# francescofrontera/flink-jpmml

Measured on AMD Instinct MI355X. Metric: records/sec (whole node) on 1k-tree GBDT PMML at 1/2/4/8 MI355X; p50 latency, higher is better.
Workload: dtype fp32

## Files before the change

### flink_jpmml_amd/config.py

```python

from __future__ import annotations

import dataclasses
import os
from dataclasses import dataclass, field
from typing import Any, Dict, Optional, Sequence

PRECISIONS = ("fp32", "bf16", "fp8")
FALLBACKS = ("host", "warn", "error")


@dataclass
class ScoringConfig:
    batch_size: Optional[int] = None
    """Flush a per-record micro-batch once it holds this many records (``None`` = score each record
    as it arrives, exactly the reference's call pattern)."""
    udf_mode: str = "deferred"
    """How a micro-batched per-record UDF is run: ``deferred`` — exactly once per event, its
    ``predict`` calls resolved when the batch is scored; ``replay`` — capture, batch score, replay
    (the UDF runs twice: pure UDFs that read the score inside ``f`` batch fully)."""
    max_batch_latency_ms: Optional[float] = None
    """Flush a non-empty micro-batch once its oldest record has waited this long (size-or-time
    trigger). ``None`` = size, control message, checkpoint barrier or end of input only."""

# ... 11 lines not shown
    """What happens when a model cannot be lowered to the device: ``host`` — score on the host
    oracle (batched, vectorised) and count ``scoring.host_fallback``; ``warn`` — the same plus one
    WARNING per model; ``error`` — fail the model load (strict production setting)."""

    reason_codes: bool = False
    """Rank a Scorecard's ``reasonCode`` Output fields (rank 1 … 8) on the device when a batch is
    scored with ``outputs=True`` (``FJA_REASON_CODES=1``). Off: such a field does not lower, and the
    Output fields of that model follow ``fallback``. Other models ignore it."""

    entity_ranks: bool = False
    """Rank the entity Output fields of a clustering or k-NN model on the device when a batch is
    scored with ``outputs=True`` (``FJA_ENTITY_RANKS=1``): ``entityId`` / ``clusterId`` / affinity of
    rank 1 … 32, the affinity of a named cluster, the neighbours' ids and distances. Off: such a field
    does not lower, and the Output fields of that model follow ``fallback``. Other models ignore it."""

    knn_classes: bool = False
    """Score the class Output fields of a k-NN classifier on the device when a batch is scored with
    ``outputs=True`` (``FJA_KNN_CLASSES=1``): the predicted label, the vote shares as ``probability``
    and ``top_k``. Off: such a field does not lower, and the Output fields of that model follow
    ``fallback``. Other models ignore it."""

    svm_classes: bool = False
    """Score the class Output fields of an SVM classifier on the device when a batch is scored with
    ``outputs=True`` (``FJA_SVM_CLASSES=1``): the predicted label, the machines' vote shares as
    ``probability`` and ``top_k``. Off: such a field does not lower, and the Output fields of that
    model follow ``fallback``. Other models ignore it."""

    association_rules: bool = False
    """Rank the ``ruleValue`` / ``entityId`` Output fields of an AssociationModel (rank 1 … 8) on the
    device when a batch is scored with ``outputs=True`` (``FJA_ASSOCIATION_RULES=1``). Off: the
    Output fields of such a model are computed on the host, row by row. A document the rule kernel
    cannot take follows ``fallback``. Other models ignore it."""

    host_threads: int = 0
    """Worker threads of the native host tree walk (``fallback="host"`` models, CPU-only ranks,
    direct CPU ``predict_batch``); 0 = ``FJA_HOST_THREADS`` or 1. Results do not depend on it."""

    micro_batch: int = 1 << 19
    """Rows per device kernel launch when a RecordBatch is split (H2D / kernel overlap)."""
    pipeline_depth: int = 3
    """Device input slots of the H2D → kernel ring (copy of batch i+1 overlaps kernel i)."""
    h2d_streams: int = 0
    """Copy streams each micro-batch's host→device transfer is split over (concurrent copy
    engines); 0 = calibrate 1 vs 2 on the first copy and keep the faster (boxes differ)."""
    max_inflight: int = 4
    """Scored batches an operator keeps in flight before it waits for the oldest (backpressure)."""
    metrics_port: int = 0
    """> 0: every rank serves its metrics in the Prometheus text format on ``GET /metrics`` at
    ``metrics_port + rank`` (127.0.0.1) while a job runs (``utils/metrics.py``)."""
    graph_max_rows: int = 16384
    """Micro-batches of at most this many rows run multi-kernel plans (wide NeuralNetworks,
    segmented ensembles, derive pass + model) as one HIP-graph replay per row bucket
    (:mod:`flink_jpmml_amd.runtime.graphs`); 0 = always launch kernel by kernel."""
    device_mirror: bool = False
    """Keep ``[rows]`` device copies of every columnar result (``PredictionBatch.device_out``) next
    to the pinned host scores, so a :class:`~flink_jpmml_amd.parallel.sinks.GatherSink` all-gathers
    them over RCCL without a host round trip (SURVEY §2.6 F5)."""

    cache_capacity: int = 64
    """Exact-key LRU capacity of loaded models per operator instance."""
    async_load: bool = True
    """Parse + lower an added model on a background loader thread (the event path only waits if an
    event needs the model before the load finished)."""

    checkpoint_dir: Optional[str] = None
    watchdog_s: Optional[float] = None
    """Arm a progress watchdog in the distributed loop: abort the rank when no element was processed
    for this long (a peer stuck in a collective cannot be interrupted from Python)."""

    plan_opts: Dict[str, Any] = field(default_factory=dict)
    """Extra lowering options forwarded to :func:`flink_jpmml_amd.runtime.plans.compile_plan`."""

    def __post_init__(self) -> None:
        if self.precision not in PRECISIONS:
            raise ValueError(f"precision must be one of {PRECISIONS}, got {self.precision!r}")
        if self.udf_mode not in ("deferred", "replay"):
            raise ValueError(f"udf_mode must be 'deferred' or 'replay', got {self.udf_mode!r}")
        if self.fallback not in FALLBACKS:
            raise ValueError(f"fallback must be one of {FALLBACKS}, got {self.fallback!r}")
        if self.batch_size is not None and int(self.batch_size) < 1:
            raise ValueError("batch_size must be >= 1")
        if self.max_batch_latency_ms is not None and float(self.max_batch_latency_ms) < 0:
            raise ValueError("max_batch_latency_ms must be >= 0")
        if self.micro_batch < 1 or self.pipeline_depth < 1 or self.max_inflight < 1:
            raise ValueError("micro_batch, pipeline_depth and max_inflight must be >= 1")

    def replace(self, **kw) -> "ScoringConfig":
        return dataclasses.replace(self, **{k: v for k, v in kw.items() if v is not None})

    def lowering_opts(self) -> Dict[str, Any]:
        opts = dict(self.plan_opts)
        if self.precision != "fp32":
            opts.setdefault("precision", self.precision)
        return opts

    def resolve_device(self, local_rank: int = 0):
        if self.device is None:
            return None
        import torch

        if isinstance(self.device, str) and self.device == "auto":
            if not torch.cuda.is_available():
                return None
            dev = torch.device("cuda")
        else:
            dev = torch.device(self.device) if not isinstance(self.device, torch.device) else self.device
        if dev.type != "cuda":
            return None if dev.type == "cpu" else dev
        if self.device_ids is not None:
            return torch.device("cuda", int(self.device_ids[local_rank % len(self.device_ids)]))
        if dev.index is None:
            n = max(1, torch.cuda.device_count())
            return torch.device("cuda", local_rank % n)
        return dev

    @staticmethod
    def from_env(prefix: str = "FJA_", **overrides) -> "ScoringConfig":
        def get(name, conv):
            v = os.environ.get(prefix + name)
            return conv(v) if v not in (None, "") else None

        kw = dict(batch_size=get("BATCH_SIZE", int), max_batch_latency_ms=get("MAX_BATCH_LATENCY_MS", float),
                  device=get("DEVICE", str), precision=get("PRECISION", str), fallback=get("FALLBACK", str),
                  micro_batch=get("MICRO_BATCH", int), cache_capacity=get("CACHE_CAPACITY", int),
                  checkpoint_dir=get("CHECKPOINT_DIR", str), watchdog_s=get("WATCHDOG_S", float),
                  graph_max_rows=get("GRAPH_MAX_ROWS", int), metrics_port=get("METRICS_PORT", int),
                  host_threads=get("HOST_THREADS", int),
                  reason_codes=get("REASON_CODES", lambda v: v.strip().lower() in ("1", "true", "yes", "on")),
                  entity_ranks=get("ENTITY_RANKS", lambda v: v.strip().lower() in ("1", "true", "yes", "on")),
                  knn_classes=get("KNN_CLASSES", lambda v: v.strip().lower() in ("1", "true", "yes", "on")),
                  svm_classes=get("SVM_CLASSES", lambda v: v.strip().lower() in ("1", "true", "yes", "on")),
                  association_rules=get("ASSOCIATION_RULES",
                                        lambda v: v.strip().lower() in ("1", "true", "yes", "on")))
        kw = {k: v for k, v in kw.items() if v is not None}
        kw.update({k: v for k, v in overrides.items() if v is not None})
        return ScoringConfig(**kw)


def merge_config(config: Optional[ScoringConfig], **legacy) -> ScoringConfig:
    base = config if config is not None else ScoringConfig()
    kw = {k: v for k, v in legacy.items() if v is not None}
    if "plan_opts" in kw:
        kw["plan_opts"] = {**base.plan_opts, **kw["plan_opts"]}
    return dataclasses.replace(base, **kw) if kw else base


__all__ = ["FALLBACKS", "PRECISIONS", "ScoringConfig", "merge_config"]
```

### flink_jpmml_amd/ops/_lib.py

```python

from __future__ import annotations

import ctypes
import glob
import logging
import os
import shutil
import subprocess
import threading
import time
from typing import List, Optional

logger = logging.getLogger(__name__)

HERE = os.path.dirname(os.path.abspath(__file__))
CSRC = os.path.join(HERE, "csrc")
LIB_PATH = os.path.join(HERE, "_pmml_kernels.so")
ARCH = os.environ.get("PYTORCH_ROCM_ARCH", "gfx950").split(";")[0] or "gfx950"


class KernelLibraryError(RuntimeError):
    pass


# ... 342 lines not shown
        lib.pmml_gemm_fused_head_launch.restype = ctypes.c_int
        lib.pmml_gemm_fused_head_launch.argtypes = [c_void_p, ctypes.POINTER(GemmArgs), ctypes.POINTER(GemmArgs),
                                                    c_void_p, c_void_p]
        lib.pmml_nn_prep_launch.restype = ctypes.c_int
        lib.pmml_nn_prep_launch.argtypes = [c_void_p, ctypes.POINTER(NnPrepArgs)]
        lib.pmml_knn_launch.restype = ctypes.c_int
        lib.pmml_knn_launch.argtypes = [c_void_p, ctypes.POINTER(KnnArgs), c_void_p, c_void_p, ctypes.c_int,
                                        ctypes.c_int]
        lib.pmml_linear_launch.argtypes = [c_void_p, ctypes.POINTER(LinearArgs)]
        if hasattr(lib, "pmml_mlp_launch"):
            lib.pmml_mlp_launch.argtypes = [c_void_p, ctypes.POINTER(MlpArgs), c_int]
        if hasattr(lib, "pmml_svm_launch"):
            lib.pmml_svm_launch.argtypes = [c_void_p, ctypes.POINTER(SvmArgs), c_int, c_int]
        if hasattr(lib, "pmml_svm_wide_launch"):
            lib.pmml_svm_wide_launch.restype = c_int
            lib.pmml_svm_wide_launch.argtypes = [c_void_p, ctypes.POINTER(SvmWideArgs), c_int, c_int]
        lib.pmml_tree_general_launch.argtypes = [c_void_p, ctypes.POINTER(GenTreeArgs)]
        lib.pmml_tree_general_launch.restype = c_int
        lib.pmml_tree_hybrid_launch.argtypes = [c_void_p, ctypes.POINTER(HybridArgs), c_int, c_int]
        lib.pmml_tree_hybrid_launch.restype = c_int
        lib.pmml_derive_launch.argtypes = [c_void_p, ctypes.POINTER(DeriveArgs)]
        lib.pmml_derive_launch.restype = c_int
        lib.pmml_mask_invalid.argtypes = [c_void_p, c_void_p, c_void_p, c_void_p, c_void_p, c_void_p, c_int]
        lib.pmml_mask_invalid.restype = c_int
        lib.pmml_host_register.argtypes = [c_void_p, ctypes.c_size_t, ctypes.c_uint]
        lib.pmml_host_register.restype = c_int
        lib.pmml_host_unregister.argtypes = [c_void_p]
        lib.pmml_host_unregister.restype = c_int
        lib.pmml_segment_reduce.argtypes = [c_void_p, ctypes.POINTER(SegArgs)]
        lib.pmml_tree_pointer_multi.argtypes = [c_void_p, ctypes.POINTER(MultiTreeArgs), c_int, c_int]
        lib.pmml_tree_pointer_multi.restype = c_int
        lib.pmml_segment_reduce.restype = c_int
        lib.pmml_tree_launch_many.argtypes = [c_void_p, c_void_p, c_void_p, c_int]
        lib.pmml_tree_launch_many.restype = c_int
        lib.pmml_text_rows_count.argtypes = [c_void_p, c_void_p, ctypes.c_longlong, c_void_p]
        lib.pmml_text_rows_count.restype = c_int
        lib.pmml_text_rows_write.argtypes = [c_void_p, c_void_p, ctypes.c_longlong, c_void_p, c_void_p]
        lib.pmml_text_rows_write.restype = c_int
        lib.pmml_text_parse.argtypes = [c_void_p, ctypes.POINTER(TextParseArgs)]
        lib.pmml_text_parse.restype = c_int
        lib.pmml_group_rows.argtypes = [c_void_p, c_void_p, c_int, c_int, c_int, c_void_p, c_int, c_int, c_void_p,
                                        c_void_p, c_void_p]
        lib.pmml_group_rows.restype = c_int
        lib.pmml_ungroup.argtypes = [c_void_p, c_void_p, c_void_p, c_void_p, c_int, c_void_p, c_void_p, c_void_p,
                                     c_void_p]
        lib.pmml_ungroup.restype = c_int
        lib.pmml_group_slice.argtypes = [c_void_p, c_void_p, c_int, c_int, c_int, c_void_p, c_int, c_int, c_void_p,
                                         c_void_p, c_int, c_void_p, c_void_p, c_void_p, c_void_p, c_void_p,
                                         c_void_p, c_void_p, c_void_p, c_void_p]
        lib.pmml_group_slice.restype = c_int
        lib.pmml_tree_launch_grouped.argtypes = [c_void_p, c_void_p, c_int, ctypes.POINTER(GroupedTreeArgs), c_int,
                                                 c_int]
        lib.pmml_tree_launch_grouped.restype = c_int
        lib.pmml_tree_lds_launch.argtypes = [c_void_p, ctypes.POINTER(LdsTreeArgs)]
        lib.pmml_tree_lds_launch.restype = c_int
        lib.pmml_tree_lds_bytes.argtypes = [c_int, c_int, c_int, c_int, c_int]
        lib.pmml_tree_lds_bytes.restype = ctypes.c_longlong
        lib.pmml_csr_expand.argtypes = [c_void_p, ctypes.POINTER(CsrExpandArgs)]
        lib.pmml_csr_expand.restype = c_int
        lib.pmml_csr_expand_rows.argtypes = [c_int]
        lib.pmml_csr_expand_rows.restype = c_int
        lib.pmml_outputs_launch.argtypes = [c_void_p, ctypes.POINTER(OutputArgs)]
        lib.pmml_outputs_launch.restype = c_int
        lib.pmml_outputs_rows.argtypes = [c_int, c_int]
        lib.pmml_outputs_rows.restype = c_int
        lib.pmml_reasons_launch.argtypes = [c_void_p, ctypes.POINTER(ReasonArgs)]
        lib.pmml_reasons_launch.restype = c_int
        lib.pmml_reasons_lds_bytes.argtypes = [c_int, c_int, c_int, c_int, c_int]
        lib.pmml_reasons_lds_bytes.restype = ctypes.c_longlong
        lib.pmml_entities_launch.argtypes = [c_void_p, ctypes.POINTER(EntityArgs)]
        lib.pmml_entities_launch.restype = c_int
        lib.pmml_entities_lds_bytes.argtypes = [c_int, c_int, c_int]
        lib.pmml_entities_lds_bytes.restype = ctypes.c_longlong
        lib.pmml_rules_launch.argtypes = [c_void_p, ctypes.POINTER(RuleArgs)]
        lib.pmml_rules_launch.restype = c_int
        lib.pmml_rules_lds_bytes.argtypes = [c_int, c_int, c_int]
        lib.pmml_rules_lds_bytes.restype = ctypes.c_longlong
        _lib = lib
        return lib


def check(rc: int, what: str) -> None:
    if rc != 0:
        raise KernelLibraryError(f"{what} failed with code {rc}")


def ptr(t) -> Optional[int]:
    if t is None:
        return None
    return t.data_ptr()


def stream_handle(stream=None) -> int:
    import torch

    s = stream if stream is not None else torch.cuda.current_stream()
    return s.cuda_stream


def host_device_ptr(t) -> Optional[int]:
    if t is None or not t.is_pinned():
        return None
    lib = load()
    dev = c_void_p()
    rc = lib.pmml_host_device_ptr(c_void_p(t.data_ptr()), ctypes.byref(dev))
    if rc != 0 or not dev.value:
# ... 3 lines not shown
```

### flink_jpmml_amd/runtime/engine.py

```python

from __future__ import annotations

import collections
import logging
import threading
import time
from dataclasses import dataclass
from typing import Tuple, List, Optional

import numpy as np

from ..api.batch import PredictionBatch, RecordBatch, SparseRecordBatch
from ..ops.sparse import MAX_WIDTH as CSR_MAX_WIDTH
from ..utils.metrics import METRICS
from ..utils.profiling import prange

logger = logging.getLogger(__name__)


@dataclass
class StepHandle:
    n: int
    done: object
    score_dev: object = None
    valid_dev: object = None
    out_index: int = 0


SPLIT_COPY_MIN_BYTES = 8 << 20


class DevicePipeline:

    def __init__(self, device, micro_batch: int = 1 << 19, depth: int = 3, h2d_streams: int = 0):
        import torch

        self.device = torch.device(device)
        self.B = int(micro_batch)
        self.depth = int(depth)
        self.auto_h2d = int(h2d_streams) <= 0
        self.h2ds = [torch.cuda.Stream(self.device) for _ in range(2 if self.auto_h2d else int(h2d_streams))]
        self.n_h2d = None if self.auto_h2d else len(self.h2ds)
        self.h2d = self.h2ds[0]
        self.comp = torch.cuda.Stream(self.device)
        self.d2h = torch.cuda.Stream(self.device)
        self.slot_elems = 0
        self.slots: List = []
        self.ev_h2d = [[torch.cuda.Event() for _ in self.h2ds] for _ in range(self.depth)]
        self.ev_comp = [torch.cuda.Event() for _ in range(self.depth)]
        self.used = [False] * self.depth
        self.next = 0
        self._dev_ptr_cache = {}
        self.csr: List = [None] * self.depth

    def ensure_slots(self, elems: int) -> None:
        if elems <= self.slot_elems:
            return
        import torch

        for t in self.slots:
            t.record_stream(self.comp)
            for st in self.h2ds:
                t.record_stream(st)
        self.slots = [torch.empty(elems, dtype=torch.float32, device=self.device) for _ in range(self.depth)]
        self.slot_elems = elems

    def ensure_csr(self, slot: int, rows: int, nnz: int):
        import torch

        cur = self.csr[slot]
        if cur is not None and cur[0].numel() >= rows + 1 and cur[1].numel() >= nnz:
            return cur
        if cur is not None:
            for t in cur:
                t.record_stream(self.comp)
                for st in self.h2ds:
                    t.record_stream(st)
            rows, nnz = max(rows, cur[0].numel() - 1), max(nnz, cur[1].numel())
        cap = max(1024, nnz + (nnz >> 2))
        cur = [torch.empty(max(rows, self.B) + 1, dtype=torch.int32, device=self.device),
               torch.empty(cap, dtype=torch.int32, device=self.device),
               torch.empty(cap, dtype=torch.float32, device=self.device)]
        self.csr[slot] = cur
        return cur

    @property
    def h2d_streams_in_use(self) -> Optional[int]:
        return self.n_h2d

    def active_h2d(self) -> List:
        if self.n_h2d is None:
            self.n_h2d = self._calibrate_h2d()
        return self.h2ds[: self.n_h2d]

    def _calibrate_h2d(self, mib: int = 128, reps: int = 3) -> int:
        import time

        import torch

        n = mib * (1 << 18)
        src = torch.empty(n, dtype=torch.float32, pin_memory=True)
        src.fill_(1.0)
        dst = torch.empty(n, dtype=torch.float32, device=self.device)
        best = {}
        for k in (1, 2):
            part = -(-n // k)
# ... 16 lines not shown
        METRICS.observe("pipeline.h2d_streams_chosen", float(choice))
        return choice

    def host_dev_ptr(self, t):
        from ..ops._lib import host_device_ptr

        key = (t.data_ptr(), t.numel())
        p = self._dev_ptr_cache.get(key)
        if p is None:
            p = host_device_ptr(t)
            if len(self._dev_ptr_cache) > 4096:
                self._dev_ptr_cache.clear()
            self._dev_ptr_cache[key] = p
        return p


def _pin(X):
    import torch

    if isinstance(X, torch.Tensor):
        src = X.to(torch.float32).contiguous()
    else:
        src = torch.from_numpy(np.ascontiguousarray(X, dtype=np.float32))
    out = torch.empty(src.shape, dtype=torch.float32, pin_memory=True)
    out.copy_(src)
    return out


def _pin_as(a: np.ndarray, dtype):
    import torch

    src = torch.from_numpy(np.ascontiguousarray(a))
    out = torch.empty(src.shape, dtype=dtype, pin_memory=True)
    out.copy_(src)
    return out


@dataclass
class _CsrSource:
    batch: object
    indptr: np.ndarray
    rebased: object
    indices: object
    values: object
    fill: float


class StreamingScorer:
    kind = "device"

    def __init__(self, plan, micro_batch: int = 131072, depth: int = 3, max_rows: Optional[int] = None,
                 out_buffers: int = 2, direct_host_output: bool = True, keep_device_output: bool = True,
                 h2d_streams: int = 0, pipeline: Optional[DevicePipeline] = None, max_inflight: int = 4,
                 graph_max_rows: int = 0):
        self.plan = plan
        self.device = plan.device
        self.F = plan.n_features
        self.pipe = pipeline if pipeline is not None else DevicePipeline(self.device, micro_batch, depth, h2d_streams)
        self.B = self.pipe.B
        self.depth = self.pipe.depth
        self.h2ds, self.h2d, self.comp, self.d2h = self.pipe.h2ds, self.pipe.h2d, self.pipe.comp, self.pipe.d2h
        self.max_rows = max_rows or self.B
        self.n_out = int(out_buffers)
        self._outs = None
        self._out_free: List[Optional[object]] = [None] * self.n_out
        self._out_i = 0
        self.batch_times_ms: List[float] = []
        self.direct = bool(direct_host_output) and getattr(plan, "supports_direct", False)
        self.keep_device = keep_device_output
        self.max_inflight = int(max_inflight)
        self._inflight: "collections.deque" = collections.deque()
        self.rows_submitted = 0
        self._out_plans: dict = {}
        self._out_lock = threading.Lock()
        self.fallback = "warn"
        self.lowering_opts: dict = {}
        self.reason_codes = False
        self.entity_ranks = False
        self.knn_classes = False
        self.svm_classes = False
        self._row_state = None
        self._row_lock = threading.Lock()
        from ..ops import _lib

        self._lib = _lib.load()
        self._graphs = None
        if graph_max_rows > 0 and getattr(plan, "graph_small_batches", False):
            from .graphs import GraphLauncher

            self._graphs = GraphLauncher(plan, max_rows=graph_max_rows)

    def _alloc_out(self, n: int):
        import torch

        return (torch.empty(n, dtype=torch.float32, device=self.device),
                torch.empty(n, dtype=torch.uint8, device=self.device))

    @property
    def score_dev(self):
        self.ensure_capacity(0)
        return self._outs[(self._out_i - 1) % self.n_out][0]

    @property
    def valid_dev(self):
        self.ensure_capacity(0)
        return self._outs[(self._out_i - 1) % self.n_out][1]

    def ensure_capacity(self, n: int) -> None:
        if n > self.max_rows or self._outs is None:
            if self._outs is not None:
                for pair in self._outs:
                    for t in pair:
                        t.record_stream(self.comp)
            self.max_rows = max(n, self.max_rows)
            self._outs = [self._alloc_out(self.max_rows) for _ in range(self.n_out)]
            self._out_free = [None] * self.n_out

    def _slot(self, m: int):
        p = self.pipe
        p.ensure_slots(p.B * max(self.F, 1))
        slot = p.next
        p.next = (slot + 1) % p.depth
        return slot, p.slots[slot][: m * self.F].view(m, self.F)

    def _enqueue(self, X_src, s: int, e: int, out_score, out_valid, kw) -> None:
        import torch

        p = self.pipe
        m = e - s
        if X_src.is_cuda:
            xs, slot = X_src[s:e], None
        else:
            slot, xs = self._slot(m)
            h2ds = p.active_h2d()
            if len(h2ds) > 1 and m * self.F * 4 < SPLIT_COPY_MIN_BYTES:
                h2ds = h2ds[:1]
            part = -(-m // len(h2ds))
            raw = X_src.is_contiguous() and X_src.dtype == torch.float32
            if raw:
                rowb = self.F * 4
                src0, dst0 = X_src.data_ptr() + s * rowb, xs.data_ptr()
            for j, st in enumerate(h2ds):
                if p.used[slot]:
# ... 94 lines not shown

    @staticmethod
    def wait(handle: StepHandle) -> None:
        handle.done.synchronize()

    def _throttle(self) -> None:
        while len(self._inflight) >= self.max_inflight:
            self._inflight.popleft()[0].synchronize()
        while self._inflight and self._inflight[0][0].query():
            self._inflight.popleft()

    def _output_plan(self, top_k: int):
        op = self._out_plans.get(top_k)
        if op is not None:
            return op
        with self._out_lock:
            op = self._out_plans.get(top_k)
            if op is None:
                op = self._out_plans[top_k] = self._lower_outputs(top_k)
        return op

    def _lower_outputs(self, top_k: int):
        from .plans import NotLowerable

        compiled = getattr(self.plan, "compiled", None)
        if compiled is None or not hasattr(compiled, "output_plan"):
            from ..api.exceptions import UnsupportedFeatureException

            raise UnsupportedFeatureException(
                "Output fields need the PMML document: this scorer's plan arrived by replication "
                "without it (bind the model from its document on this rank)")
        try:
            return compiled.output_plan(self.device, top_k=top_k, reason_codes=self.reason_codes,
                                        entity_ranks=self.entity_ranks, knn_classes=self.knn_classes,
                                        svm_classes=self.svm_classes, **self.lowering_opts)
        except NotLowerable as e:
            if self.fallback == "error":
                raise
            METRICS.inc("scoring.host_fallback_outputs")
            if self.fallback == "warn":
                logger.warning("Output fields of model %r cannot run on %s (%s): computing them on the "
                               "host oracle (set fallback='error' to refuse)", compiled.model_name, self.device, e)
            return HostScorer(compiled, reason=str(e))

    def submit_batch(self, batch: RecordBatch, replace_nan: Optional[float] = None,
                     keep_device: bool = False, outputs: bool = False, top_k: int = 0) -> PredictionBatch:
        import torch

        n = len(batch)
        if n == 0:
            return PredictionBatch.empty(0)
        if batch.n_features != self.F:
            raise ValueError(f"batch has {batch.n_features} features, model expects {self.F}")
        op = None
        if outputs:
            op = self._output_plan(int(top_k))
            if isinstance(op, HostScorer):
                return op.submit_batch(batch, replace_nan, outputs=True, top_k=top_k)
        if isinstance(batch, SparseRecordBatch) and self.F <= CSR_MAX_WIDTH:
            return self._submit(batch, self._stage_csr(batch, replace_nan), self._enqueue_csr, keep_device, op)
        X = batch.X
        if replace_nan is not None:
            Xn = np.array(batch.numpy(), dtype=np.float32, copy=True)
            Xn[batch.absent if batch.absent is not None else np.isnan(Xn)] = replace_nan
            X = Xn
        with prange("score.stage"):
            if not isinstance(X, torch.Tensor):
                X = _pin(X)
            elif X.is_cuda:
                if X.dtype != torch.float32 or not X.is_contiguous():
                    X = X.to(torch.float32).contiguous()
                if getattr(batch, "ready", None) is not None:
                    self.comp.wait_event(batch.ready)
                else:
                    self.comp.wait_stream(torch.cuda.current_stream(self.device))
                X.record_stream(self.comp)
            elif not X.is_pinned() or X.dtype != torch.float32 or not X.is_contiguous():
                X = _pin(X)
        return self._submit(batch, X, self._enqueue, keep_device, op)

    def _submit(self, batch: RecordBatch, X, enqueue, keep_device: bool, out_plan=None) -> PredictionBatch:
        import torch

        n = len(batch)
        self._throttle()
        score_h = torch.empty(n, dtype=torch.float32, pin_memory=True)
        valid_h = torch.empty(n, dtype=torch.uint8, pin_memory=True)
        dev_out = None
        hs = hv = None
        out_h = out_d = None
        if self.direct and out_plan is None:
            hs, hv = self.pipe.host_dev_ptr(score_h), self.pipe.host_dev_ptr(valid_h)
            if hs is None or hv is None:
                hs = hv = None
        if keep_device or hs is None:
            with torch.cuda.stream(self.comp):
                dev_out = (torch.empty(n, dtype=torch.float32, device=self.device),
                           torch.empty(n, dtype=torch.uint8, device=self.device))
        if out_plan is not None:
            out_h = torch.empty((n, out_plan.width), dtype=torch.float32, pin_memory=True)
            with torch.cuda.stream(self.comp):
                out_d = torch.empty((n, out_plan.width), dtype=torch.float32, device=self.device)
        with prange("score.enqueue"):
            for s in range(0, n, self.B):
                e = min(n, s + self.B)
                if hs is not None:
                    kw = dict(score2=dev_out[0][s:e], valid2=dev_out[1][s:e]) if dev_out is not None else {}
                    enqueue(X, s, e, hs + 4 * s, hv + s, kw)
                elif out_plan is not None:
                    enqueue(X, s, e, dev_out[0][s:e], dev_out[1][s:e], dict(outputs=out_d[s:e], plan=out_plan))
                else:
                    enqueue(X, s, e, dev_out[0][s:e], dev_out[1][s:e], {})
            done = torch.cuda.Event()
            if hs is None:
                ev = torch.cuda.Event()
                ev.record(self.comp)
                with torch.cuda.stream(self.d2h):
                    self.d2h.wait_event(ev)
                    score_h.copy_(dev_out[0], non_blocking=True)
                    valid_h.copy_(dev_out[1], non_blocking=True)
                    if out_d is not None:
                        out_h.copy_(out_d, non_blocking=True)
                        out_d.record_stream(self.d2h)
                    for t in dev_out:
                        t.record_stream(self.d2h)
                done.record(self.d2h)
            else:
                done.record(self.comp)
        self._inflight.append((done, X))
        self.rows_submitted += n
        METRICS.inc("scoring.rows_device", n)
        METRICS.inc("scoring.batches_device")
# ... 217 lines not shown
def _rule_plan(compiled, device, cfg):
    from ..models.association import AssociationEvaluator
    from .plans import NotLowerable

    if device is None or not cfg.association_rules or not isinstance(compiled.evaluator, AssociationEvaluator):
        return None
    try:
        with prange("model.lower"):
            return compiled.output_plan(device, association_rules=True, **cfg.lowering_opts())
    except NotLowerable as e:
        if cfg.fallback == "error":
            from ..api.exceptions import ModelLoadingException

            raise ModelLoadingException(f"Output fields of model {compiled.model_name!r} are not lowerable to "
                                        f"{device}: {e}", e) from e
        METRICS.inc("scoring.host_fallback_outputs")
        if cfg.fallback == "warn":
            logger.warning("Output fields of model %r cannot run on %s (%s): computing them on the "
                           "host oracle (set fallback='error' to refuse)", compiled.model_name, device, e)
        return None


def make_scorer(compiled, device, config=None, pipeline: Optional[DevicePipeline] = None, plan=None,
                lower_error: Optional[str] = None):
    from ..config import ScoringConfig
    from .plans import NotLowerable

    cfg = config or ScoringConfig()
    if not compiled.target_fields:
        return NullScorer(compiled.n_features, compiled, _rule_plan(compiled, device, cfg))
    if cfg.host_threads:
        _set_host_threads(cfg.host_threads)
    if device is None:
        return HostScorer(compiled)
    if plan is None:
        try:
            if lower_error is not None:
                raise NotLowerable(lower_error)
            with prange("model.lower"):
                plan = compiled.plan(device, **cfg.lowering_opts())
        except NotLowerable as e:
            if cfg.fallback == "error":
                from ..api.exceptions import ModelLoadingException

                raise ModelLoadingException(f"model {compiled.model_name!r} is not lowerable to {device}: {e}",
                                            e) from e
            METRICS.inc("scoring.host_fallback_models")
            if cfg.fallback == "warn":
                logger.warning("model %r cannot run on %s (%s): scoring it on the host oracle "
                               "(set fallback='error' to refuse)", compiled.model_name, device, e)
            return HostScorer(compiled, reason=str(e))
    if pipeline is None:
        pipeline = DevicePipeline(plan.device, cfg.micro_batch, cfg.pipeline_depth, cfg.h2d_streams)
    scorer = StreamingScorer(plan, pipeline=pipeline, max_inflight=cfg.max_inflight, graph_max_rows=cfg.graph_max_rows)
    scorer.fallback, scorer.lowering_opts = cfg.fallback, dict(cfg.lowering_opts())
    scorer.reason_codes = bool(cfg.reason_codes)
    scorer.entity_ranks = bool(cfg.entity_ranks)
    scorer.knn_classes = bool(cfg.knn_classes)
    scorer.svm_classes = bool(cfg.svm_classes)
    return scorer


__all__ = ["DevicePipeline", "HostScorer", "NullScorer", "StepHandle", "StreamingScorer", "make_scorer"]
```

### flink_jpmml_amd/runtime/plans.py

```python

from __future__ import annotations

import collections
import dataclasses
import logging
import math
import threading
from dataclasses import dataclass
from typing import Any, List, Optional, Tuple

import numpy as np

from ..api.exceptions import UnsupportedFeatureException
from ..models.clustering import ClusteringEvaluator
from ..models.mining import MiningEvaluator
from ..models.regression import RegressionEvaluator
from ..models.tree import OP_GE, OP_GT, OP_LE, OP_LT, BinaryTree, NotBinary, TreeEvaluator, lower_binary_tree
from ..pmml import ir

logger = logging.getLogger(__name__)

TB = 256

FP_HAS_MISSING_REPL = 1 << 0
# ... 1606 lines not shown
                if prep[j, 0] & (FP_INVALID_RETURN | FP_ROW_INVALID | FP_INTEGER | FP_CODE_RANGE | FP_HAS_INTERVAL | FP_VALUE_MASK):
                    used.add(j)
        return sorted(used) if used else [0]

    def _vote_mode(self, spec, rows) -> int:
        G = 1024 // (rows or 256)
        unweighted = spec.tree_w is None or all(w == 1.0 for w in spec.tree_w)
        no_nan = all(not np.isnan(t.leaf_value[t.feature < 0]).any() for t in spec.trees)
        if unweighted and spec.C <= 4 and no_nan and -(-len(spec.trees) // G) <= 255:
            return 3
        return 2

    def _chunk(self, fit: int, wide: bool, cap: int, slot_cap: int = 0) -> int:
        c = int(max(1, min(self.n_trees, fit)))
        if slot_cap:
            c = min(c, slot_cap)
        G = 1024 // self.rows_wide
        if wide and c < self.n_trees:
            q = DYN_B if slot_cap else (8 * G if c >= 16 * G else 2 * G)
            c = max(q, c // q * q) if c >= q else c
        return min(c, cap) if cap > 0 else c

    @staticmethod
    def _general_spec(compiled) -> "EnsembleSpec":
        from .general_tree import lower_general_tree

        try:
            spec = ensemble_spec(compiled, lower=lower_general_tree)
            if spec.mode == "slot" and any(b != 0.0 for b in (spec.acc_init or [])):
                raise NotLowerable("K-class chains with intercepts over non-binary trees are host-only")
            for i, t in enumerate(spec.trees):
                if getattr(t, "mix_mass", None) is None:
                    continue
                if spec.mode == "class":
                    t.mix_vote, t.mix_weight = True, float((spec.tree_w or [1.0] * len(spec.trees))[i])
                elif spec.mode == "sum" and spec.P > 1 and spec.slots is None:
                    t.mix_vote, t.mix_weight = False, float(spec.weights[i])
                else:
                    raise NotLowerable("sibling mixture trees inside this ensemble form are host-only")
                cats = list(spec.labels or [])
                tc = list(t.ev.categories)
                if any(c not in cats for c in tc):
                    raise NotLowerable("tree category outside the ensemble's classes")
                t.mix_remap = np.array([cats.index(c) for c in tc], dtype=np.int32)
            return to_general(spec)
        except NotBinary as e:
            raise NotLowerable(str(e)) from e

    def _post_state(self) -> None:
        self._partial = None
        self._retired = []
        self._args = {}
        self._args_buf = {}

    def _args_template(self, with_probs: bool):
        import ctypes

        from ..ops._lib import TreeArgs, ptr

        cache = self._args
        a = cache.get(with_probs)
        if a is None:
            a = TreeArgs()
            a.prep = ptr(self.prep)
            a.blob, a.roots, a.leaves, a.tree_slot = ptr(self.blob), ptr(self.roots), ptr(self.leaves), ptr(self.slots)
            a.n_trees, a.rec_words, a.chunk_trees, a.P = self.n_trees, self.rec_words, self.chunk_trees, self.P
            a.C, a.general, a.variant = self.C, self.general, self.variant
            a.blob_nan, a.chunk_trees_nan = ptr(self.blob_nan), self.chunk_trees_nan
            a.tree_w, a.acc_init, a.feat_map = ptr(self.tree_w), ptr(self.acc_init), ptr(self.feat_map)
            a.rows_wide, a.mode, a.n_stage, a.pilp = self.rows_wide, self.mode, self.n_stage, self.pointer_ilp
            a.prof = ptr(self.prof)
            a.rank_thr, a.rank_cnt, a.rank_stride = ptr(self.rank_thr), ptr(self.rank_cnt), int(self.rank_stride)
            a.leaf_onehot = int(self.leaf_onehot)
            a.epi = _epilogue(table=self.table, write_probs=with_probs, **self.epi_args)
            cache[with_probs] = a
        bufs = self._args_buf
        key = (threading.get_ident(), with_probs)
        b = bufs.get(key)
        if b is None:
            if len(bufs) > 64:
                bufs.clear()
            b = bufs[key] = TreeArgs()
        ctypes.pointer(b)[0] = a
        return b

    def _auto_splits(self, n_rows: int) -> int:
        if self.splits:
            return self.splits
        blocks = (n_rows + TB - 1) // TB
        if self.xcd_split and self.n_trees >= 2 * XCD_SLICES:
            return XCD_SLICES
        if self.layout == "perfect" and self.variant & 3 and self.n_trees >= 64:
            return int(max(1, min(16, 256 // max(1, blocks), self.n_trees // 8)))
        target = 512
        if blocks >= target or self.n_trees < 64:
            return 1
        return int(max(1, min(self.n_trees // 16, target // max(1, blocks), 64)))

    supports_direct = True

    def _bind_rows(self, a, x_ptr, n: int, n_feat: int, ldx: int, score, valid, s: int = 1, row_valid=None,
                   probs=None, score2=None, valid2=None) -> None:
        a.X, a.n_rows, a.n_feat, a.ldx = x_ptr, n, n_feat, ldx
        a.row_valid_in = row_valid
        a.score, a.valid, a.probs = score, valid, probs
        a.epi.score2, a.epi.valid2 = score2, valid2
# ... 34 lines not shown
            return
        if self.layout == "hybrid":
            from ..ops._lib import HybridArgs

            h = HybridArgs()
            h.t = a
            h.heads, h.head_words, h.tail_format = ptr(self.heads), int(self.rec_words), int(self.tail_format)
            rc = self.lib.pmml_tree_hybrid_launch(stream_handle(stream), ctypes.byref(h), int(self.head_depth), s)
            check(rc, f"tree kernel (hybrid, head {self.head_depth}, depth {self.depth})")
            return
        rc = self.lib.pmml_tree_launch(stream_handle(stream), ctypes.byref(a), 0 if self.layout == "perfect" else 1,
                                       self.depth, 1 if self.has_dr else 0, s)
        check(rc, f"tree kernel ({self.layout}, depth {self.depth})")

    def row_launcher(self, X, score, valid):
        if self.layout not in ("perfect", "pointer") or self.variant & VAR_POINTER_LDS or X.shape[1] == 0:
            return None
        import ctypes

        import torch

        from ..ops._lib import TreeArgs, check, stream_handle

        n = X.shape[0]
        s = self._auto_splits(n)
        a = TreeArgs()
        ctypes.memmove(ctypes.byref(a), ctypes.byref(self._args_template(False)), ctypes.sizeof(TreeArgs))
        self._bind_rows(a, X.data_ptr(), n, X.shape[1], X.stride(0), _addr(score), _addr(valid), s)
        partial = None
        if s > 1:
            partial = torch.empty(max(s * (self.C + 1) * n, 1), dtype=torch.float32, device=self.device)
            a.partial = partial.data_ptr()
        lib, layout = self.lib, 0 if self.layout == "perfect" else 1
        depth, dr = self.depth, 1 if self.has_dr else 0

        def run(stream) -> None:
            check(lib.pmml_tree_launch(stream_handle(stream), ctypes.byref(a), layout, depth, dr, s),
                  f"tree kernel ({self.layout}, depth {depth}, row)")

        run.keep = (a, partial, X)
        return run

    def batch_launch_args(self, x_ptr: int, n: int, n_feat: int, ldx: int, score_ptr: int, valid_ptr: int):
        from ..ops._lib import TreeArgs

        if self.layout not in ("perfect", "pointer") or n <= 0 or self.variant & VAR_POINTER_LDS:
            return None
        s = self._auto_splits(n)
        a = TreeArgs.from_buffer_copy(self._args_template(False))
        self._bind_rows(a, x_ptr, n, n_feat, ldx, score_ptr, valid_ptr, s)
        if s > 1:
            a.partial = self._shared_partial(s * (self.C + 1) * n)
        return a, (0 if self.layout == "perfect" else 1, int(self.depth), 1 if self.has_dr else 0, int(s))

    def grouped_args(self, n_feat: int):
        from ..ops._lib import TreeArgs

        if self.layout != "perfect" or not (self.variant & 3) or self.P != 1 or self.n_stage > n_feat:
            return None
        a = TreeArgs.from_buffer_copy(self._args_template(False))
        a.X, a.n_rows, a.n_feat, a.ldx = None, 0, n_feat, n_feat
        a.row_valid_in, a.score, a.valid, a.probs, a.partial, a.prof = None, None, None, None, None, None
        a.epi.score2, a.epi.valid2 = None, None
        a.xcd_split, a.trees_per_split = 0, self.n_trees
        rows = int(a.rows_wide)
        return a, int(self.depth), (int(self.depth), int(self.variant & 3), rows, int(a.mode)), rows

    def _launch_general(self, X, score, valid, stream, probs, row_valid, score2, valid2) -> None:
        import ctypes

        from ..ops._lib import GenTreeArgs, check, ptr, stream_handle

        g = GenTreeArgs()
        g.t = self._args_template(probs is not None)
        self._bind_rows(g.t, X.data_ptr(), X.shape[0], X.shape[1], X.stride(0), _addr(score), _addr(valid), 1,
                        ptr(row_valid), ptr(probs), _addr(score2), _addr(valid2))
        g.nodes, g.children, g.preds = ptr(self.blob), ptr(self.children), ptr(self.preds)
        g.pool, g.trees, g.max_steps = ptr(self.pool), ptr(self.trees_tab), int(self.max_steps)
        g.mix_mass, g.mix_w = ptr(self.mix_mass), ptr(self.mix_w)
        g.mix_tab, g.remap, g.vcol = ptr(self.mix_tab), ptr(self.mix_remap), ptr(self.vcol)
        check(self.lib.pmml_tree_general_launch(stream_handle(stream), ctypes.byref(g)), "general tree kernel")




def _segmented_plan(compiled, device, fused_error: Exception, opts: dict) -> DevicePlan:
    from .segmented import ChainPlan, SegmentedPlan, segmentable

    ev = compiled.evaluator
    if getattr(ev, "method", None) == "modelChain":
        try:
            return _with_prepared_inputs(compiled, device, lambda c: ChainPlan(c, device, **opts), opts)
        except NotLowerable as e:
            raise NotLowerable(f"{fused_error}; modelChain: {e}") from e
    why = segmentable(compiled.evaluator, compiled)
    if why:
        raise NotLowerable(f"{fused_error}; segmentation: {why}") from fused_error
    return _with_prepared_inputs(compiled, device, lambda c: SegmentedPlan(c, device, **opts), opts)


def _with_prepared_inputs(compiled, device, build, opts: dict) -> DevicePlan:
    if not getattr(compiled, "prepared_inputs", False):
        _, any_prep = build_field_prep(compiled, compiled.active_fields) if compiled.active_fields \
            else (None, False)
        if any_prep:
            from .derive import DerivedPlan, build_program_layout
# ... 101 lines not shown
```

Baseline: 439.0 million.

## Add native single-call request path for small pinned tree-model batches

Adds a native C++ request object that does the H2D copy, tree kernel launch and completion event in one call on the compute stream. Small pinned fp32 RecordBatches of tree models skip the Python streaming pipeline, copy stream and cross-stream hand-over. This is meant to cut per-batch host and synchronisation overhead for small batches. The cost is a second code path with its own device buffer and cached args, plus an event ring of 64 that could alias if more than 64 requests are in flight.

```diff
diff --git a/flink_jpmml_amd/config.py b/flink_jpmml_amd/config.py
--- a/flink_jpmml_amd/config.py
+++ b/flink_jpmml_amd/config.py
@@ -87,6 +87,12 @@
     """Micro-batches of at most this many rows run multi-kernel plans (wide NeuralNetworks,
     segmented ensembles, derive pass + model) as one HIP-graph replay per row bucket
     (:mod:`flink_jpmml_amd.runtime.graphs`); 0 = always launch kernel by kernel."""
+    native_requests: bool = True
+    """Score a small pinned fp32 ``RecordBatch`` (at most ``micro_batch`` rows and under the
+    small-copy threshold of 8 MiB) of a tree model in one native call on the compute stream — copy,
+    launch and completion event, no copy stream or cross-stream hand-over
+    (:mod:`flink_jpmml_amd.runtime.request`). Same kernels and the same bits as the streaming path,
+    which ``False`` forces for every batch."""
     device_mirror: bool = False
     """Keep ``[rows]`` device copies of every columnar result (``PredictionBatch.device_out``) next
     to the pinned host scores, so a :class:`~flink_jpmml_amd.parallel.sinks.GatherSink` all-gathers
@@ -166,7 +172,8 @@
                   knn_classes=get("KNN_CLASSES", lambda v: v.strip().lower() in ("1", "true", "yes", "on")),
                   svm_classes=get("SVM_CLASSES", lambda v: v.strip().lower() in ("1", "true", "yes", "on")),
                   association_rules=get("ASSOCIATION_RULES",
-                                        lambda v: v.strip().lower() in ("1", "true", "yes", "on")))
+                                        lambda v: v.strip().lower() in ("1", "true", "yes", "on")),
+                  native_requests=get("NATIVE_REQUESTS", lambda v: v.strip().lower() in ("1", "true", "yes", "on")))
         kw = {k: v for k, v in kw.items() if v is not None}
         kw.update({k: v for k, v in overrides.items() if v is not None})
         return ScoringConfig(**kw)
diff --git a/flink_jpmml_amd/ops/_lib.py b/flink_jpmml_amd/ops/_lib.py
--- a/flink_jpmml_amd/ops/_lib.py
+++ b/flink_jpmml_amd/ops/_lib.py
@@ -418,6 +418,17 @@
         lib.pmml_tree_launch_grouped.argtypes = [c_void_p, c_void_p, c_int, ctypes.POINTER(GroupedTreeArgs), c_int,
                                                  c_int]
         lib.pmml_tree_launch_grouped.restype = c_int
+        lib.pmml_request_create.argtypes = [c_void_p, c_int, ctypes.c_size_t, ctypes.POINTER(c_void_p)]
+        lib.pmml_request_create.restype = c_int
+        lib.pmml_request_destroy.argtypes = [c_void_p]
+        lib.pmml_request_destroy.restype = c_int
+        lib.pmml_request_submit.argtypes = [c_void_p, ctypes.POINTER(TreeArgs), c_int, c_int, c_int, c_int, c_void_p,
+                                            c_int, c_void_p, c_void_p, ctypes.POINTER(ctypes.c_ulonglong)]
+        lib.pmml_request_submit.restype = c_int
+        lib.pmml_request_query.argtypes = [c_void_p, ctypes.c_ulonglong]
+        lib.pmml_request_query.restype = c_int
+        lib.pmml_request_wait.argtypes = [c_void_p, ctypes.c_ulonglong]
+        lib.pmml_request_wait.restype = c_int
         lib.pmml_tree_lds_launch.argtypes = [c_void_p, ctypes.POINTER(LdsTreeArgs)]
         lib.pmml_tree_lds_launch.restype = c_int
         lib.pmml_tree_lds_bytes.argtypes = [c_int, c_int, c_int, c_int, c_int]
diff --git a/flink_jpmml_amd/ops/csrc/request.hip b/flink_jpmml_amd/ops/csrc/request.hip
--- /dev/null
+++ b/flink_jpmml_amd/ops/csrc/request.hip
@@ -0,0 +1,110 @@
+#include <mutex>
+#include <new>
+
+#include "tree_common.h"
+
+using pmml_tree::TreeArgs;
+
+PMML_API int pmml_tree_launch(hipStream_t stream, const TreeArgs* args, int layout, int depth, int has_dr,
+                              int splits);
+
+namespace {
+
+constexpr int REQ_EVENTS = 64;
+
+struct Request {
+  hipStream_t stream = nullptr;
+  void* x_dev = nullptr;
+  size_t x_cap = 0;
+  std::mutex mu;
+  hipEvent_t ev[REQ_EVENTS] = {};
+  int n_ev = 0;
+  unsigned long long next = 1;
+};
+
+inline hipEvent_t event_of(const Request* r, unsigned long long ticket) { return r->ev[ticket % REQ_EVENTS]; }
+
+}
+
+PMML_API int pmml_request_create(hipStream_t stream, int device, size_t x_bytes_max, void** out) {
+  if (out == nullptr || x_bytes_max == 0) return (int)hipErrorInvalidValue;
+  *out = nullptr;
+  int prev = -1;
+  hipError_t e = hipGetDevice(&prev);
+  if (e != hipSuccess) return (int)e;
+  if (device >= 0 && device != prev && (e = hipSetDevice(device)) != hipSuccess) return (int)e;
+  Request* r = new (std::nothrow) Request();
+  if (r == nullptr) e = hipErrorOutOfMemory;
+  if (e == hipSuccess) {
+    r->stream = stream;
+    r->x_cap = x_bytes_max;
+    e = hipMalloc(&r->x_dev, x_bytes_max);
+  }
+  while (e == hipSuccess && r->n_ev < REQ_EVENTS) {
+    e = hipEventCreateWithFlags(&r->ev[r->n_ev], hipEventDisableTiming);
+    if (e == hipSuccess) ++r->n_ev;
+  }
+  if (e != hipSuccess && r != nullptr) {
+    for (int i = 0; i < r->n_ev; ++i) (void)hipEventDestroy(r->ev[i]);
+    if (r->x_dev) (void)hipFree(r->x_dev);
+    delete r;
+    r = nullptr;
+  }
+  if (device >= 0 && device != prev) (void)hipSetDevice(prev);
+  *out = r;
+  return (int)e;
+}
+
+PMML_API int pmml_request_destroy(void* req) {
+  Request* r = static_cast<Request*>(req);
+  if (r == nullptr) return 0;
+  hipError_t e;
+  {
+    std::lock_guard<std::mutex> lock(r->mu);
+    e = hipStreamSynchronize(r->stream);
+    for (int i = 0; i < r->n_ev; ++i) (void)hipEventDestroy(r->ev[i]);
+    if (r->x_dev) (void)hipFree(r->x_dev);
+  }
+  delete r;
+  return (int)e;
+}
+
+PMML_API int pmml_request_submit(void* req, const TreeArgs* prepared, int layout, int depth, int has_dr, int splits,
+                                 const void* x_pinned, int n, void* score_out, void* valid_out,
+                                 unsigned long long* ticket) {
+  Request* r = static_cast<Request*>(req);
+  if (r == nullptr || prepared == nullptr || x_pinned == nullptr || ticket == nullptr || n <= 0 ||
+      prepared->n_feat <= 0 || score_out == nullptr || valid_out == nullptr)
+    return (int)hipErrorInvalidValue;
+  const size_t bytes = (size_t)n * (size_t)prepared->n_feat * sizeof(float);
+  if (bytes > r->x_cap) return (int)hipErrorInvalidValue;
+  TreeArgs a = *prepared;
+  a.X = static_cast<const float*>(r->x_dev);
+  a.n_rows = n;
+  a.ldx = a.n_feat;
+  a.score = static_cast<float*>(score_out);
+  a.valid = static_cast<uint8_t*>(valid_out);
+  std::lock_guard<std::mutex> lock(r->mu);
+  hipError_t e = hipMemcpyAsync(r->x_dev, x_pinned, bytes, hipMemcpyHostToDevice, r->stream);
+  if (e != hipSuccess) return (int)e;
+  const int rc = pmml_tree_launch(r->stream, &a, layout, depth, has_dr, splits);
+  if (rc != 0) return rc;
+  const unsigned long long t = r->next;
+  e = hipEventRecord(event_of(r, t), r->stream);
+  if (e != hipSuccess) return (int)e;
+  r->next = t + 1;
+  *ticket = t;
+  return 0;
+}
+
+PMML_API int pmml_request_query(void* req, unsigned long long ticket) {
+  Request* r = static_cast<Request*>(req);
+  if (r == nullptr || ticket == 0) return (int)hipErrorInvalidValue;
+  return (int)hipEventQuery(event_of(r, ticket));
+}
+
+PMML_API int pmml_request_wait(void* req, unsigned long long ticket) {
+  Request* r = static_cast<Request*>(req);
+  if (r == nullptr || ticket == 0) return (int)hipErrorInvalidValue;
+  return (int)hipEventSynchronize(event_of(r, ticket));
+}
diff --git a/flink_jpmml_amd/runtime/engine.py b/flink_jpmml_amd/runtime/engine.py
--- a/flink_jpmml_amd/runtime/engine.py
+++ b/flink_jpmml_amd/runtime/engine.py
@@ -14,6 +14,7 @@
 from ..ops.sparse import MAX_WIDTH as CSR_MAX_WIDTH
 from ..utils.metrics import METRICS
 from ..utils.profiling import prange
+from .request import native_request_eligible
 
 logger = logging.getLogger(__name__)
 
@@ -52,6 +53,19 @@
         self.next = 0
         self._dev_ptr_cache = {}
         self.csr: List = [None] * self.depth
+        self._request = None
+        self._request_lock = threading.Lock()
+
+    def native_request(self):
+        r = self._request
+        if r is None:
+            with self._request_lock:
+                r = self._request
+                if r is None:
+                    from .request import NativeRequest
+
+                    r = self._request = NativeRequest(self.comp, self.device, SPLIT_COPY_MIN_BYTES)
+        return r
 
     def ensure_slots(self, elems: int) -> None:
         if elems <= self.slot_elems:
@@ -174,7 +188,7 @@
     def __init__(self, plan, micro_batch: int = 131072, depth: int = 3, max_rows: Optional[int] = None,
                  out_buffers: int = 2, direct_host_output: bool = True, keep_device_output: bool = True,
                  h2d_streams: int = 0, pipeline: Optional[DevicePipeline] = None, max_inflight: int = 4,
-                 graph_max_rows: int = 0):
+                 graph_max_rows: int = 0, native_requests: bool = True):
         self.plan = plan
         self.device = plan.device
         self.F = plan.n_features
@@ -211,6 +225,7 @@
             from .graphs import GraphLauncher
 
             self._graphs = GraphLauncher(plan, max_rows=graph_max_rows)
+        self.native_requests = bool(native_requests)
 
     def _alloc_out(self, n: int):
         import torch
@@ -411,6 +426,12 @@
             return PredictionBatch.empty(0)
         if batch.n_features != self.F:
             raise ValueError(f"batch has {batch.n_features} features, model expects {self.F}")
+        if self.native_requests and type(batch) is RecordBatch and native_request_eligible(
+                batch, batch.X, n, self.F, self.B, SPLIT_COPY_MIN_BYTES, replace_nan, outputs, keep_device,
+                self._graphs, self.direct, True, getattr(self.plan, "prepares_launch", False)):
+            pb = self._submit_native(batch, batch.X, n)
+            if pb is not None:
+                return pb
         op = None
         if outputs:
             op = self._output_plan(int(top_k))
@@ -437,6 +458,28 @@
             elif not X.is_pinned() or X.dtype != torch.float32 or not X.is_contiguous():
                 X = _pin(X)
         return self._submit(batch, X, self._enqueue, keep_device, op)
+
+    def _submit_native(self, batch: RecordBatch, X, n: int) -> Optional[PredictionBatch]:
+        import torch
+
+        prepared = self.plan.request_args(n, self.F)
+        if prepared is None:
+            return None
+        self._throttle()
+        score_h = torch.empty(n, dtype=torch.float32, pin_memory=True)
+        valid_h = torch.empty(n, dtype=torch.uint8, pin_memory=True)
+        hs, hv = self.pipe.host_dev_ptr(score_h), self.pipe.host_dev_ptr(valid_h)
+        if hs is None or hv is None:
+            return None
+        done = self.pipe.native_request().submit(prepared[0], prepared[1], X.data_ptr(), n, hs, hv,
+                                                 (X, score_h, valid_h))
+        self._inflight.append((done, X))
+        self.rows_submitted += n
+        METRICS.inc("scoring.rows_device", n)
+        METRICS.inc("scoring.batches_device")
+        METRICS.inc("scoring.requests_native")
+        return PredictionBatch(n, score_h, valid_h, done, owner=(X, None, None), on_done=_observe_latency,
+                               row_ok=batch.size_ok())
 
     def _submit(self, batch: RecordBatch, X, enqueue, keep_device: bool, out_plan=None) -> PredictionBatch:
         import torch
@@ -760,7 +803,8 @@
             return HostScorer(compiled, reason=str(e))
     if pipeline is None:
         pipeline = DevicePipeline(plan.device, cfg.micro_batch, cfg.pipeline_depth, cfg.h2d_streams)
-    scorer = StreamingScorer(plan, pipeline=pipeline, max_inflight=cfg.max_inflight, graph_max_rows=cfg.graph_max_rows)
+    scorer = StreamingScorer(plan, pipeline=pipeline, max_inflight=cfg.max_inflight, graph_max_rows=cfg.graph_max_rows,
+                             native_requests=cfg.native_requests)
     scorer.fallback, scorer.lowering_opts = cfg.fallback, dict(cfg.lowering_opts())
     scorer.reason_codes = bool(cfg.reason_codes)
     scorer.entity_ranks = bool(cfg.entity_ranks)
diff --git a/flink_jpmml_amd/runtime/plans.py b/flink_jpmml_amd/runtime/plans.py
--- a/flink_jpmml_amd/runtime/plans.py
+++ b/flink_jpmml_amd/runtime/plans.py
@@ -1682,6 +1682,7 @@
         self._retired = []
         self._args = {}
         self._args_buf = {}
+        self._request_args = {}
 
     def _args_template(self, with_probs: bool):
         import ctypes
@@ -1822,6 +1823,25 @@
         if s > 1:
             a.partial = self._shared_partial(s * (self.C + 1) * n)
         return a, (0 if self.layout == "perfect" else 1, int(self.depth), 1 if self.has_dr else 0, int(s))
+
+    REQUEST_ARGS_MAX = 64
+
+    @property
+    def prepares_launch(self) -> bool:
+        return self.layout in ("perfect", "pointer") and not self.variant & VAR_POINTER_LDS
+
+    def request_args(self, n: int, n_feat: int):
+        s = self._auto_splits(n)
+        cache = self._request_args
+        e = cache.get((n, s))
+        if e is None:
+            made = self.batch_launch_args(None, n, n_feat, n_feat, None, None)
+            if made is None:
+                return None
+            if len(cache) >= self.REQUEST_ARGS_MAX:
+                cache.clear()
+            e = cache[(n, s)] = (made[0], made[1], self._partial if made[1][3] > 1 else None)
+        return e
 
     def grouped_args(self, n_feat: int):
         from ..ops._lib import TreeArgs
diff --git a/flink_jpmml_amd/runtime/request.py b/flink_jpmml_amd/runtime/request.py
--- /dev/null
+++ b/flink_jpmml_amd/runtime/request.py
@@ -0,0 +1,98 @@
+
+from __future__ import annotations
+
+import ctypes
+import sys
+from typing import Any, Optional
+
+HIP_ERROR_NOT_READY = 600
+
+
+def native_request_eligible(batch: Any, X: Any, n: int, n_features: int, micro_batch: int, max_bytes: int,
+                            replace_nan: Optional[float] = None, outputs: bool = False, keep_device: bool = False,
+                            graphs: Any = None, direct: bool = True, enabled: bool = True,
+                            plan_prepares: bool = True) -> bool:
+    from ..api.batch import RecordBatch
+
+    if not (enabled and direct and plan_prepares) or graphs is not None:
+        return False
+    if replace_nan is not None or outputs or keep_device:
+        return False
+    if type(batch) is not RecordBatch:
+        return False
+    if n < 1 or n > micro_batch or n_features < 1 or n * n_features * 4 >= max_bytes:
+        return False
+    is_pinned = getattr(X, "is_pinned", None)
+    if is_pinned is None or getattr(X, "is_cuda", False):
+        return False
+    import torch
+
+    return bool(X.dtype == torch.float32 and X.is_contiguous() and is_pinned())
+
+
+class RequestDone:
+
+    __slots__ = ("_req", "_ticket", "_keep")
+
+    def __init__(self, req: "NativeRequest", ticket: int, keep: Any):
+        self._req, self._ticket, self._keep = req, ticket, keep
+
+    def synchronize(self) -> None:
+        if self._keep is None:
+            return
+        rc = self._req.lib.pmml_request_wait(self._req.handle, self._ticket)
+        self._keep = None
+        if rc != 0:
+            raise RuntimeError(f"small request failed on the device (HIP error {rc})")
+
+    def query(self) -> bool:
+        if self._keep is None:
+            return True
+        rc = self._req.lib.pmml_request_query(self._req.handle, self._ticket)
+        if rc == HIP_ERROR_NOT_READY:
+            return False
+        self._keep = None
+        if rc != 0:
+            raise RuntimeError(f"small request failed on the device (HIP error {rc})")
+        return True
+
+
+class NativeRequest:
+
+    def __init__(self, stream, device, x_bytes_max: int):
+        from ..ops import _lib
+
+        self.lib = _lib.load()
+        self.stream = stream
+        self.x_bytes_max = int(x_bytes_max)
+        h = ctypes.c_void_p()
+        index = -1 if device.index is None else int(device.index)
+        _lib.check(self.lib.pmml_request_create(stream.cuda_stream, index, self.x_bytes_max, ctypes.byref(h)),
+                   "small-request object")
+        self.handle = h
+
+    def submit(self, args, meta, x_ptr: int, n: int, score_ptr: int, valid_ptr: int, keep: Any) -> RequestDone:
+        t = ctypes.c_ulonglong()
+        rc = self.lib.pmml_request_submit(self.handle, ctypes.byref(args), meta[0], meta[1], meta[2], meta[3], x_ptr, n,
+                                          score_ptr, valid_ptr, ctypes.byref(t))
+        if rc != 0:
+            from ..ops._lib import KernelLibraryError
+
+            raise KernelLibraryError(f"small request of {n} rows failed with code {rc}")
+        return RequestDone(self, t.value, keep)
+
+    def close(self) -> None:
+        h, self.handle = self.handle, None
+        if h is not None and h.value:
+            self.lib.pmml_request_destroy(h)
+
+    def __del__(self):
+        try:
+            if sys is None or sys.is_finalizing():
+                return
+            self.close()
+        except Exception:
+            pass
+
+
+__all__ = ["HIP_ERROR_NOT_READY", "NativeRequest", "RequestDone", "native_request_eligible"]
diff --git a/profiles/small_request/measure.py b/profiles/small_request/measure.py
--- /dev/null
+++ b/profiles/small_request/measure.py
@@ -0,0 +1,138 @@
+
+import argparse
+import json
+import os
+import sys
+import time
+
+import numpy as np
+import torch
+
+ROOT = os.path.dirname(os.path.dirname(os.path.dirname(os.path.abspath(__file__))))
+if os.path.isdir(os.path.join(ROOT, "flink_jpmml_amd")) and ROOT not in sys.path:
+    sys.path.insert(0, ROOT)
+if os.getcwd() not in sys.path:
+    sys.path.insert(0, os.getcwd())
+
+from flink_jpmml_amd.api.batch import RecordBatch
+from flink_jpmml_amd.api.pmml_model import PmmlModel
+from flink_jpmml_amd.bench.synth import gbdt_pmml, stream_matrix
+from flink_jpmml_amd.config import ScoringConfig
+from flink_jpmml_amd.ops._lib import check
+
+F = 32
+SIZES = (1, 256, 1024, 4096, 16384)
+COPY_BYTES = (4 << 10, 32 << 10, 128 << 10, 512 << 10, 2 << 20)
+WARM, TIMED = 20, 500
+
+
+def pct(ts, q):
+    return round(float(np.percentile(np.asarray(ts) * 1e6, q)), 2)
+
+
+def timed(fn):
+    ts = []
+    for i in range(WARM + TIMED):
+        t0 = time.perf_counter()
+        fn()
+        if i >= WARM:
+            ts.append(time.perf_counter() - t0)
+    return ts
+
+
+def kernel_us(plan, X, stream):
+    n = X.shape[0]
+    xd = X.cuda()
+    s = torch.empty(n, dtype=torch.float32, device="cuda")
+    v = torch.empty(n, dtype=torch.uint8, device="cuda")
+    evs = [(torch.cuda.Event(enable_timing=True), torch.cuda.Event(enable_timing=True)) for _ in range(TIMED)]
+    for i in range(WARM + TIMED):
+        if i >= WARM:
+            evs[i - WARM][0].record(stream)
+        plan.launch(xd, s, v, stream=stream)
+        if i >= WARM:
+            evs[i - WARM][1].record(stream)
+    stream.synchronize()
+    return round(float(np.median([a.elapsed_time(b) for a, b in evs])) * 1e3, 2)
+
+
+def lean_us(scorer, X):
+    plan, pipe, lib = scorer.plan, scorer.pipe, scorer._lib
+    n = X.shape[0]
+    xd = torch.empty((n, F), dtype=torch.float32, device="cuda")
+    sh = torch.empty(n, dtype=torch.float32, pin_memory=True)
+    vh = torch.empty(n, dtype=torch.uint8, pin_memory=True)
+    run = plan.row_launcher(xd, pipe.host_dev_ptr(sh), pipe.host_dev_ptr(vh))
+    cs = pipe.comp.cuda_stream
+    src, dst, nbytes = X.data_ptr(), xd.data_ptr(), n * F * 4
+
+    def one():
+        check(lib.pmml_memcpy_async(dst, src, nbytes, 1, cs), "H2D")
+        run(pipe.comp)
+        pipe.comp.synchronize()
+
+    return pct(timed(one), 50)
+
+
+def copy_table(scorer):
+    import ctypes
+
+    pipe, lib = scorer.pipe, scorer._lib
+    lib.pmml_pull_copy.restype = ctypes.c_int
+    lib.pmml_pull_copy.argtypes = [ctypes.c_void_p, ctypes.c_void_p, ctypes.c_void_p, ctypes.c_size_t, ctypes.c_int]
+    cs = pipe.comp.cuda_stream
+    out = []
+    for nbytes in COPY_BYTES:
+        src = torch.empty(nbytes // 4, dtype=torch.float32, pin_memory=True)
+        src.fill_(1.0)
+        dst = torch.empty(nbytes // 4, dtype=torch.float32, device="cuda")
+        sp, sd, dp = src.data_ptr(), pipe.host_dev_ptr(src), dst.data_ptr()
+        blocks = min(1024, -(-nbytes // 16 // 256))
+
+        def memcpy():
+            check(lib.pmml_memcpy_async(dp, sp, nbytes, 1, cs), "hipMemcpyAsync")
+            pipe.comp.synchronize()
+
+        def pull():
+            check(lib.pmml_pull_copy(cs, sd, dp, nbytes, blocks), "pull copy")
+            pipe.comp.synchronize()
+
+        out.append({"bytes": nbytes, "memcpy_us": pct(timed(memcpy), 50), "pull_us": pct(timed(pull), 50)})
+        assert bool((dst == 1.0).all())
+    return out
+
+
+def main():
+    ap = argparse.ArgumentParser()
+    ap.add_argument("--out", default=os.path.join(os.path.dirname(os.path.abspath(__file__)), "results.json"))
+    a = ap.parse_args()
+    text = gbdt_pmml(n_trees=1000, depth=6, n_features=F, seed=0)
+    models = {}
+    for native in (False, True):
+        cfg = ScoringConfig(device="cuda:0", micro_batch=1 << 20, native_requests=native, fallback="error")
+        models[native] = PmmlModel.from_string(text).bind(torch.device("cuda:0"), cfg)
+    res = {"model": "GBDT 1000 trees x depth 6, 32 fp32 features", "device": torch.cuda.get_device_name(0),
+           "timed": TIMED, "warmup": WARM, "sizes": []}
+    for n in SIZES:
+        X = torch.from_numpy(stream_matrix(n, F, seed=7)).pin_memory()
+        sc = models[False].scorer
+        row = {"rows": n, "splits": sc.plan._auto_splits(n), "kernel_us": kernel_us(sc.plan, X, sc.pipe.comp),
+               "lean_us": lean_us(sc, X)}
+        for native, key in ((False, "stream"), (True, "native")):
+            m, batch = models[native], RecordBatch(X)
+            ts = timed(lambda: m.predict(batch).wait())
+            row[f"{key}_p50_us"], row[f"{key}_p99_us"] = pct(ts, 50), pct(ts, 99)
+        row["ratio_p50"] = round(row["native_p50_us"] / row["stream_p50_us"], 3)
+        print(json.dumps(row), flush=True)
+        res["sizes"].append(row)
+    res["copy"] = copy_table(models[True].scorer)
+    for r in res["copy"]:
+        print(json.dumps(r), flush=True)
+    os.makedirs(os.path.dirname(os.path.abspath(a.out)), exist_ok=True)
+    with open(a.out, "w") as fh:
+        json.dump(res, fh, indent=1)
+        fh.write("\n")
+
+
+if __name__ == "__main__":
+    main()
```

New measurement: 438.6 million. No clear change (-0.1%).
